# nekStab/neklab

Measured on AMD Instinct MI355X. Metric: linop matvecs/sec + Arnoldi iter time, E=10k N=7, 1/2/4/8 GPU, higher is better.
Workload: dtype f64

## Files before the change

neklab_amd/csrc/lns.hip:

```cpp
#include <cmath>
#include <functional>
#include <map>
#include <string>

#include "internal.h"

using namespace nlg;

namespace {

constexpr int NT = 256;
constexpr int NB = 512;

struct F3 {
    double *p[3];
};
struct CF3 {
    const double *p[3];
};
__device__ __forceinline__ int64_t lane_lo(int64_t ld) { return (int64_t)blockIdx.y * ld; }
__device__ __forceinline__ F3 lane_f3(F3 a, int64_t lo) {
#pragma unroll
    for (int c = 0; c < 3; ++c)
        if (a.p[c]) a.p[c] += lo;
// ... 2003 lines not shown
}

int begin_run(nlg_linop *op, int nl) {
    NLG_TRY(reset_state(op, nl));
    op->istep = 0;
    op->nproj = 0;
    for (int v = 0; v < kMaxLanes; ++v) op->lane_viters[v] = op->lane_piters[v] = 0;
    op->orbit_end_valid = op->upo_fdot_valid = false;
    return 0;
}

int load_state(nlg_linop *op, int lane, const nlg_vec *v, int irst) {
    nlg_mesh *m = op->mesh;
    hipStream_t st = m->ctx->stream;
    for (int c = 0; c < m->dim; ++c)
        NLG_HIP(hipMemcpyAsync(at_lane(op, op->ubuf[0][c], lane), v->vel(c, irst), sizeof(double) * (size_t)m->lvn, hipMemcpyDeviceToDevice, st));
    NLG_HIP(hipMemcpyAsync(at_lane(op, op->p, lane), v->pr(irst), sizeof(double) * (size_t)m->lpn, hipMemcpyDeviceToDevice, st));
    if (op->cfg.ifheat)
        NLG_HIP(hipMemcpyAsync(at_lane(op, op->tbuf[0], lane), v->theta(0, irst), sizeof(double) * (size_t)m->lvn, hipMemcpyDeviceToDevice, st));
    return 0;
}

int store_state(nlg_linop *op, int lane, nlg_vec *v, int irst) {
    nlg_mesh *m = op->mesh;
    hipStream_t st = m->ctx->stream;
    for (int c = 0; c < m->dim; ++c)
        NLG_HIP(hipMemcpyAsync(v->vel(c, irst), at_lane(op, op->ubuf[0][c], lane), sizeof(double) * (size_t)m->lvn, hipMemcpyDeviceToDevice, st));
    NLG_HIP(hipMemcpyAsync(v->pr(irst), at_lane(op, op->p, lane), sizeof(double) * (size_t)m->lpn, hipMemcpyDeviceToDevice, st));
    if (op->cfg.ifheat)
        NLG_HIP(hipMemcpyAsync(v->theta(0, irst), at_lane(op, op->tbuf[0], lane), sizeof(double) * (size_t)m->lvn, hipMemcpyDeviceToDevice, st));
    return 0;
}

int state_minus_x0(nlg_linop *op, int lane, double c, nlg_vec *out) {
    nlg_mesh *m = op->mesh;
    const int dim = m->dim;
    DdtArgs A;
    memset(&A, 0, sizeof(A));
    for (int f = 0; f <= dim; ++f) {
        const bool pr = f == dim;
        A.out[f] = pr ? out->pr() : out->vel(f), A.n[f] = pr ? m->lpn : m->lvn;
        A.src[f][0] = at_lane(op, pr ? op->p : op->ubuf[0][f], lane), A.c[f][0] = c;
        A.src[f][1] = pr ? op->baseflow->pr() : op->baseflow->vel(f), A.c[f][1] = -c;
    }
    NLG_LAUNCH(k_bdf_ddt, dim3(grid_for(m->lvn), dim + 1), dim3(NT), 0, m->ctx->stream, A);
    NLG_HIP(hipGetLastError());
    return 0;
}

enum { FDOT_START = 0, FDOT_PRE, FDOT_END };
int capture_fdot(nlg_linop *op, int lane, int phase) {
    nlg_mesh *m = op->mesh;
    const int dim = m->dim;
    const double idt = 1.0 / op->dt;
    if (phase == FDOT_START) return state_minus_x0(op, lane, idt, op->upo_f0);
    nlg_vec *o = op->upo_fT;
    DdtArgs A;
    memset(&A, 0, sizeof(A));
    for (int c = 0; c < dim; ++c) A.out[c] = o->vel(c), A.n[c] = m->lvn;
    A.out[dim] = o->pr(), A.n[dim] = m->lpn;
    if (phase == FDOT_PRE) {
        const int k = std::min(op->nsteps, op->cfg.torder);
        for (int c = 0; c < dim; ++c)
            for (int j = 0; j < k; ++j) A.src[c][j] = at_lane(op, op->ubuf[j][c], lane), A.c[c][j] = -BDF_C[k][j] * idt;
    } else {
        const int k = std::min(op->nsteps, op->cfg.torder);
// ... 68 lines not shown
    for (int v = 0; v < s; ++v) {
        NLG_CHECK(vin[v] && vout[v] && vin[v]->mesh == m && vout[v]->mesh == m, "exptA block matvec: vector %d NULL or on a different mesh", v);
        NLG_CHECK(vin[v]->nscal == want_scal && vout[v]->nscal == want_scal, "exptA block matvec: vector %d carries %d scalars, the operator %d", v,
                  vin[v]->nscal, want_scal);
        NLG_CHECK(op->cfg.no_history || (vin[v]->lorder >= op->cfg.torder && vout[v]->lorder >= op->cfg.torder), "exptA block matvec: vector lorder < time order");
        for (int u = 0; u < s; ++u) NLG_CHECK(vin[v] != vout[u], "exptA block matvec: an input vector is also an output vector");
        for (int u = 0; u < v; ++u) NLG_CHECK(vout[v] != vout[u], "exptA block matvec: the same output vector twice");
    }
    const int nrst = op->cfg.no_history ? 0 : op->cfg.torder - 1;
    const int nl = op->orbit ? s + 1 : s, lb = op->orbit ? s : -1;
    NLG_CHECK(op->proj_lanes == 0 || s <= op->proj_lanes, "exptA block matvec: %d vectors on an operator with %d wavenumber lanes (nlg_linop_set_projection_lanes)", s,
              op->proj_lanes);
    const unsigned all = (1u << s) - 1u;
    NLG_TRY(begin_run(op, nl));
    for (int v = 0; v < s; ++v) NLG_TRY(load_state(op, v, vin[v], 0));
    NLG_TRY(project_alpha(op, s, 0, all));
    if (lb >= 0) NLG_TRY(load_state(op, lb, op->baseflow, 0));
    Lanes L{op, nl, lb};
    L.adjoint = adjoint;
    NLG_TRY(run_steps(L, lb, [&](int istep) -> int {
        if (istep <= nrst) {
            unsigned replayed = 0;
            for (int v = 0; v < s; ++v)
                if (vin[v]->nrst > 0) {
                    NLG_TRY(load_state(op, v, vin[v], istep));
                    replayed |= 1u << v;
                }
            if (replayed) NLG_TRY(project_alpha(op, s, 0, replayed));
        }
        return 0;
    }));
    for (int slot = 0; slot < 3; ++slot) NLG_TRY(project_alpha(op, s, slot, all));
    for (int v = 0; v < s; ++v) {
        NLG_TRY(nlg_vec_zero(vout[v]));
        NLG_TRY(store_state(op, v, vout[v], 0));
    }
    if (lb >= 0) {
        NLG_TRY(nlg_vec_zero(op->orbit_end));
        NLG_TRY(store_state(op, lb, op->orbit_end, 0));
        op->orbit_end_valid = true;
    }
    for (int irst = 1; irst <= nrst; ++irst) {
        NLG_TRY(advance(L));
        for (int v = 0; v < s; ++v) {
            NLG_TRY(store_state(op, v, vout[v], irst));
            vout[v]->nrst = std::max(vout[v]->nrst, irst);
        }
    }
    op->st_matvecs += s;
    return 0;
}

int do_matvec(nlg_linop *op, const nlg_vec *vin, nlg_vec *vout, int adjoint) {
    NLG_CHECK(op && vin && vout, "exptA matvec: NULL argument");
    NLG_CHECK(op->inited, "exptA matvec: nlg_linop_init has not been called (reference: exptA%%init(), 1cyl.usr:20)");
    nlg_mesh *m = op->mesh;
    NLG_CHECK(vin->mesh == m && vout->mesh == m,
              "exptA matvec: vector on a different mesh (reference: type_error, exponential_propagator.f90:53-58)");
    NLG_CHECK(vin->nscal == (op->cfg.ifheat ? 1 : 0) && vout->nscal == vin->nscal,
              "exptA matvec: the vectors carry %d scalar(s), the operator expects %d (cfg.ifheat)", vin->nscal, op->cfg.ifheat ? 1 : 0);
    NLG_CHECK(op->cfg.no_history || (vin->lorder >= op->cfg.torder && vout->lorder >= op->cfg.torder),
              "exptA matvec: vector lorder %d < time order %d", vin->lorder, op->cfg.torder);
    NLG_CHECK(vin != vout, "exptA matvec: vec_in and vec_out must be distinct (intent(in) / intent(out))");
    return do_matvec_block(op, 1, &vin, &vout, adjoint);
}

int do_integrate_forced_block(nlg_linop *op, int s, const nlg_vec *const *ic, const nlg_vec *const *f_re, const nlg_vec *const *f_im, double omega,
                              int adjoint, nlg_vec *const *vout) {
    NLG_CHECK(op && f_re && vout, "integrate_forced: NULL argument");
    NLG_CHECK(s >= 1 && s <= kMaxLanes, "integrate_forced: %d forcings unsupported (1..%d)", s, kMaxLanes);
    NLG_CHECK(op->inited, "integrate_forced: nlg_linop_init has not been called");
    NLG_NO_OTD(op, "integrate_forced");
    NLG_CHECK(!op->orbit, "integrate_forced: not available in orbit mode (the forced response about a time-periodic base flow is not built; nlg_linop_set_orbit)");
    NLG_CHECK(op->proj_lanes == 0, "integrate_forced: not available on an operator with wavenumber lanes (a forced run does not project; nlg_linop_set_projection_lanes)");
    nlg_mesh *m = op->mesh;
    Lanes L{op, s};
    for (int v = 0; v < s; ++v) {
        NLG_CHECK(f_re[v] && vout[v], "integrate_forced: NULL argument (forcing or output of lane %d)", v);
        L.f_re[v] = f_re[v];
        L.f_im[v] = f_im ? f_im[v] : nullptr;
    }
    for (int v = 0; v < s; ++v) {
        const nlg_vec *icv = ic ? ic[v] : nullptr;
        NLG_CHECK(L.f_re[v]->mesh == m && vout[v]->mesh == m && (!icv || icv->mesh == m) && (!L.f_im[v] || L.f_im[v]->mesh == m),
                  "integrate_forced: vector on a different mesh");
        for (int u = 0; u < s; ++u)
            NLG_CHECK(vout[v] != L.f_re[u] && vout[v] != L.f_im[u] && !(ic && vout[v] == ic[u]), "integrate_forced: the output must be distinct from the inputs");
        for (int u = 0; u < v; ++u) NLG_CHECK(vout[v] != vout[u], "integrate_forced: the same output vector twice");
        NLG_CHECK(L.f_re[v]->nscal == 0 && vout[v]->nscal == 0, "integrate_forced: scalar (temperature) coupling is not built yet");
    }
    hipStream_t st = m->ctx->stream;
    NLG_TRY(begin_run(op, s));
    for (int v = 0; v < s; ++v) {
        NLG_HIP(hipMemsetAsync(at_lane(op, op->p, v), 0, sizeof(double) * (size_t)m->lps, st));
        if (ic && ic[v]) NLG_TRY(load_state(op, v, ic[v], 0));
    }
    L.adjoint = adjoint;
    L.omega = omega, L.sign = adjoint ? -1.0 : 1.0;
    NLG_TRY(run_steps(L));
    for (int v = 0; v < s; ++v) {
        NLG_TRY(nlg_vec_zero(vout[v]));
        NLG_TRY(store_state(op, v, vout[v], 0));
    }
    return 0;
}

int do_integrate_forced(nlg_linop *op, const nlg_vec *ic, const nlg_vec *f_re, const nlg_vec *f_im, double omega, int adjoint, nlg_vec *vout) {
    NLG_CHECK(op && f_re && vout, "integrate_forced: NULL argument");
    return do_integrate_forced_block(op, 1, &ic, &f_re, &f_im, omega, adjoint, &vout);
}

int do_nonlinear_map(nlg_linop *op, const nlg_vec *vin, nlg_vec *vout) {
    NLG_CHECK(op && vin && vout, "nonlinear_map: NULL argument");
    NLG_NO_OTD(op, "nonlinear_map");
    nlg_mesh *m = op->mesh;
    NLG_CHECK(vin->mesh == m && vout->mesh == m, "nonlinear_map: vector on a different mesh (reference: type_error, fixed_point.f90:31-36)");
    NLG_CHECK(vin->nscal == (op->cfg.ifheat ? 1 : 0) && vout->nscal == vin->nscal,
              "nonlinear_map: the vectors carry %d scalar(s), the operator expects %d (cfg.ifheat)", vin->nscal, op->cfg.ifheat ? 1 : 0);
    NLG_CHECK(vin != vout, "nonlinear_map: vec_in and vec_out must be distinct");
    NLG_CHECK(!op->orbit, "nonlinear_map: the operator is in orbit mode and holds X0 as its base flow (use a second operator, or nlg_linop_set_orbit(op, NULL, 0))");
    NLG_TRY(nlg_vec_copy(op->baseflow, vin));
    NLG_TRY(nlg_linop_init(op));
    NLG_TRY(begin_run(op, 1));
    NLG_TRY(load_state(op, 0, vin, 0));
    Lanes L{op, 1};
    L.nonlinear = 1;
    NLG_TRY(run_steps(L));
    NLG_TRY(nlg_vec_zero(vout));
    NLG_TRY(store_state(op, 0, vout, 0));
    NLG_TRY(nlg_vec_axpby(-1.0, vin, 1.0, vout));
    return 0;
}

}

namespace nlg {
int linop_proj_lanes(const nlg_linop *op) { return op->proj_lanes; }
}

extern "C" {

int nlg_exptA_config_default(nlg_exptA_config *c) {
    NLG_CHECK(c, "nlg_exptA_config_default: NULL");
    memset(c, 0, sizeof(*c));
    c->tau = 1.0;
    c->re = 100.0;
    c->cfl_limit = 0.5;
    c->vtol = 1e-9;
    c->ptol = 1e-7;
    c->dt = 0.0;
    c->torder = 3;
    c->maxit_v = 200;
    c->maxit_p = 2000;
    c->ifheat = 0;
    c->conductivity = 1.0;
    c->rhocp = 1.0;
    c->pproj = 1;
    c->no_history = 0;
    c->filter_weight = 0.0;
    c->filter_modes = 0;
    return 0;
// ... 747 lines not shown
```

neklab_amd/csrc/vec.hip:

```cpp
#include <algorithm>

#include "internal.h"

using namespace nlg;

namespace {

constexpr int NT = 256;

__device__ __forceinline__ double wave_sum(double v) {
#pragma unroll
    for (int o = 32; o > 0; o >>= 1) v += __shfl_down(v, o, 64);
    return v;
}

__device__ __forceinline__ double block_sum(double v, double *sm) {
    v = wave_sum(v);
    const int lane = threadIdx.x & 63, wid = threadIdx.x >> 6;
    __syncthreads();
    if (lane == 0) sm[wid] = v;
    __syncthreads();
    double r = 0.0;
    if (threadIdx.x == 0) {
        const int nw = (blockDim.x + 63) >> 6;
        for (int i = 0; i < nw; ++i) r += sm[i];
    }
    return r;
}

__global__ __launch_bounds__(NT) void k_fill(double2 *x, double v, int64_t n2) {
    for (int64_t i = blockIdx.x * (int64_t)NT + threadIdx.x; i < n2; i += (int64_t)gridDim.x * NT) x[i] = make_double2(v, v);
}

__global__ __launch_bounds__(NT) void k_copy(double2 *y, const double2 *x, int64_t n2) {
    for (int64_t i = blockIdx.x * (int64_t)NT + threadIdx.x; i < n2; i += (int64_t)gridDim.x * NT) y[i] = x[i];
}

__global__ __launch_bounds__(NT) void k_scal(double2 *x, double a, int64_t n2) {
    for (int64_t i = blockIdx.x * (int64_t)NT + threadIdx.x; i < n2; i += (int64_t)gridDim.x * NT) {
        double2 v = x[i];
        v.x = __dmul_rn(v.x, a);
        v.y = __dmul_rn(v.y, a);
        x[i] = v;
    }
}

struct LaneVW {
    const double *V[kMaxLanes];
    double *w[kMaxLanes];
    int nrst[kMaxLanes];
};
struct LaneAB {
    const double *a[kMaxLanes], *b[kMaxLanes];
};

__global__ __launch_bounds__(NT) void k_scal_dev(LaneVW P, const double *q, int64_t n2) {
    const int l = blockIdx.y;
    const double sv = q[l];
    const double a = sv > 0.0 ? 1.0 / sqrt(sv) : 0.0;
    const int64_t n2all = n2 * (1 + P.nrst[l]);
    double2 *x = reinterpret_cast<double2 *>(P.w[l]);
    for (int64_t i = blockIdx.x * (int64_t)NT + threadIdx.x; i < n2all; i += (int64_t)gridDim.x * NT) {
        double2 v = x[i];
        v.x = __dmul_rn(v.x, a);
        v.y = __dmul_rn(v.y, a);
        x[i] = v;
    }
}

__global__ __launch_bounds__(NT) void k_axpby(double2 *y, const double2 *x, double a, double b, int64_t n2,
                                              int nrst, int64_t blk2, int consistent) {
    for (int64_t i = blockIdx.x * (int64_t)NT + threadIdx.x; i < n2; i += (int64_t)gridDim.x * NT) {
        const double2 xv = x[i];
        const double ax0 = __dmul_rn(a, xv.x), ax1 = __dmul_rn(a, xv.y);
        double2 yv = y[i];
        yv.x = __dadd_rn(__dmul_rn(yv.x, b), ax0);
        yv.y = __dadd_rn(__dmul_rn(yv.y, b), ax1);
        y[i] = yv;
        for (int r = 1; r <= nrst; ++r) {
            double2 rv = y[i + r * blk2];
            double s0 = ax0, s1 = ax1;
            if (consistent) {
                const double2 xr = x[i + r * blk2];
                s0 = __dmul_rn(a, xr.x);
                s1 = __dmul_rn(a, xr.y);
            }
            rv.x = __dadd_rn(__dmul_rn(rv.x, b), s0);
            rv.y = __dadd_rn(__dmul_rn(rv.y, b), s1);
            y[i + r * blk2] = rv;
        }
    }
}

// ... 30 lines not shown
    const double2 *f2 = reinterpret_cast<const double2 *>(f0 + off);
    const double2 *m2 = reinterpret_cast<const double2 *>(bm1);
    double acc = 0.0;
    for (int64_t i = beg + threadIdx.x; i < end; i += NT) {
        const double2 vv = v2[i], tv = t2[i];
        double2 wv = w2[i];
        wv.x = __dadd_rn(__dadd_rn(wv.x, -vv.x), __dmul_rn(t, tv.x));
        wv.y = __dadd_rn(__dadd_rn(wv.y, -vv.y), __dmul_rn(t, tv.y));
        w2[i] = wv;
        if (ip) {
            const double2 fv = f2[i], mv = m2[i];
            acc += vv.x * fv.x * mv.x + vv.y * fv.y * mv.y;
        }
    }
    if (ip) {
        const double s = block_sum(acc, sm);
        if (threadIdx.x == 0) partial[c * nblk + blockIdx.x] = s;
    }
}

__global__ __launch_bounds__(NT) void k_reduce_rows(const double *partial, int nper, double *out, int accumulate,
                                                    double *out2) {
    __shared__ double sm[4];
    const double *p = partial + (int64_t)blockIdx.x * nper;
    double acc = 0.0;
    for (int i = threadIdx.x; i < nper; i += NT) acc += p[i];
    const double s = block_sum(acc, sm);
    if (threadIdx.x == 0) {
        out[blockIdx.x] = s;
        if (accumulate) out2[blockIdx.x] += s;
    }
}

template <int KB>
__global__ __launch_bounds__(NT) void k_block_dot(LaneVW P, int64_t vstride, int k, int ncomp, const double *bm1, int64_t lvs, int nblk,
                                                  int nper, double *partial) {
    __shared__ double sm[4 * KB];
    const int l = blockIdx.y / ncomp, c = blockIdx.y - l * ncomp;
    const double *V = P.V[l];
    const double *w = P.w[l];
    const int j0 = blockIdx.z * KB;
    const int kc = (k - j0 < KB) ? (k - j0) : KB;
    const int64_t n2 = lvs >> 1;
    const int64_t per = (n2 + nblk - 1) / nblk;
    const int64_t beg = blockIdx.x * per, end = (beg + per < n2) ? beg + per : n2;
    const double2 *w2 = reinterpret_cast<const double2 *>(w + c * lvs);
    const double2 *m2 = reinterpret_cast<const double2 *>(bm1);
    const double2 *v2[KB];
#pragma unroll
    for (int j = 0; j < KB; ++j) {
        const int jj = (j < kc) ? j : 0;
        v2[j] = reinterpret_cast<const double2 *>(V + (int64_t)(j0 + jj) * vstride + c * lvs);
    }
    double acc[KB];
#pragma unroll
    for (int j = 0; j < KB; ++j) acc[j] = 0.0;
    for (int64_t i = beg + threadIdx.x; i < end; i += NT) {
        const double2 wv = w2[i], mv = m2[i];
        const double x0 = wv.x * mv.x, x1 = wv.y * mv.y;
        double2 vv[KB];
#pragma unroll
        for (int j = 0; j < KB; ++j) vv[j] = v2[j][i];
#pragma unroll
        for (int j = 0; j < KB; ++j) acc[j] += vv[j].x * x0 + vv[j].y * x1;
    }
    const int lane = threadIdx.x & 63, wid = threadIdx.x >> 6;
#pragma unroll
    for (int j = 0; j < KB; ++j) {
        const double s = wave_sum(acc[j]);
        if (lane == 0) sm[wid * KB + j] = s;
    }
    __syncthreads();
    if (threadIdx.x < kc) {
        const int j = threadIdx.x;
        const double s = sm[j] + sm[KB + j] + sm[2 * KB + j] + sm[3 * KB + j];
        partial[((int64_t)l * k + j0 + j) * nper + c * nblk + blockIdx.x] = s;
    }
}

template <int KMAX>
__global__ __launch_bounds__(NT) void k_block_axpy_dot(const double *__restrict__ V, int64_t vstride, int k,
                                                       const double *__restrict__ h, double *__restrict__ w,
                                                       const double *__restrict__ bm1, int64_t lvs, int64_t nv,
                                                       double *__restrict__ partial) {
    __shared__ double sh[KMAX];
    __shared__ double sm[4][KMAX];
    for (int j = threadIdx.x; j < KMAX; j += NT) sh[j] = j < k ? h[j] : 0.0;
    __syncthreads();
    double acc[KMAX];
#pragma unroll
    for (int j = 0; j < KMAX; ++j) acc[j] = 0.0;
    for (int64_t i = blockIdx.x * (int64_t)NT + threadIdx.x; i < nv; i += (int64_t)gridDim.x * NT) {
        double v[KMAX];
#pragma unroll
        for (int j = 0; j < KMAX; ++j) v[j] = j < k ? V[(int64_t)j * vstride + i] : 0.0;
        double s = 0.0;
#pragma unroll
        for (int j = 0; j < KMAX; ++j) s += sh[j] * v[j];
        const double wn = w[i] - s;
        w[i] = wn;
        const double x = wn * bm1[i % lvs];
#pragma unroll
        for (int j = 0; j < KMAX; ++j) acc[j] += v[j] * x;
    }
    const int lane = threadIdx.x & 63, wid = threadIdx.x >> 6;
#pragma unroll
    for (int j = 0; j < KMAX; ++j) {
        const double t = wave_sum(acc[j]);
        if (lane == 0) sm[wid][j] = t;
// ... 27 lines not shown
        double s1 = 0.0;
#pragma unroll
        for (int j = 0; j < KH; ++j) {
            s1 += sh[KH + j] * v[j];
            mine[j * NT] = v[j];
        }
#pragma unroll
        for (int j = 0; j < KH; ++j) v[j] = V[(int64_t)j * vstride + i];
        double s0 = 0.0;
#pragma unroll
        for (int j = 0; j < KH; ++j) s0 += sh[j] * v[j];
        const double wn = w[i] - (s0 + s1);
        w[i] = wn;
        const double x = wn * bm1[i % lvs];
#pragma unroll
        for (int j = 0; j < KH; ++j) {
            acc0[j] += v[j] * x;
            acc1[j] += mine[j * NT] * x;
        }
    }
    const int lane = threadIdx.x & 63, wid = threadIdx.x >> 6;
#pragma unroll
    for (int j = 0; j < KH; ++j) {
        const double t0 = wave_sum(acc0[j]), t1 = wave_sum(acc1[j]);
        if (lane == 0) sm[wid][j] = t0, sm[wid][KH + j] = t1;
    }
    __syncthreads();
    if (threadIdx.x < k) {
        const int j = threadIdx.x;
        partial[(int64_t)j * gridDim.x + blockIdx.x] = (sm[0][j] + sm[1][j]) + (sm[2][j] + sm[3][j]);
    }
}

enum { HIST_NONE = 0, HIST_SWEEP = 1, HIST_MAIN = 2 };
__global__ __launch_bounds__(NT) void k_block_axpy(LaneVW P, int64_t vstride, int k, const double *h, const double *hh, int64_t n2,
                                                   int hist, double sign) {
    extern __shared__ double sh0[];
    double *sh1 = sh0 + k;
    const int l = blockIdx.y;
    h += (int64_t)l * k;
    if (hh) hh += (int64_t)l * k;
    for (int j = threadIdx.x; j < k; j += NT) {
        sh0[j] = h[j];
        sh1[j] = hh ? hh[j] : h[j];
    }
    __syncthreads();
    const int64_t n2all = hist == HIST_SWEEP ? n2 * (1 + P.nrst[l]) : n2;
    const int ncopy = hist == HIST_MAIN ? P.nrst[l] : 0;
    double2 *w2 = reinterpret_cast<double2 *>(P.w[l]);
    const double2 *V2 = reinterpret_cast<const double2 *>(P.V[l]);
    const int64_t vs2 = vstride >> 1;
    for (int64_t i = blockIdx.x * (int64_t)NT + threadIdx.x; i < n2all; i += (int64_t)gridDim.x * NT) {
        const double *sh = (hh && i >= n2) ? sh1 : sh0;
        double s0 = 0.0, s1 = 0.0;
        const double2 *v = V2 + i;
        int j = 0;
        for (; j + 8 <= k; j += 8) {
            double2 t[8];
#pragma unroll
            for (int u = 0; u < 8; ++u) t[u] = v[(int64_t)(j + u) * vs2];
#pragma unroll
            for (int u = 0; u < 8; ++u) {
                s0 += sh[j + u] * t[u].x;
                s1 += sh[j + u] * t[u].y;
            }
        }
        for (; j < k; ++j) {
            const double2 t = v[(int64_t)j * vs2];
            s0 += sh[j] * t.x;
            s1 += sh[j] * t.y;
        }
        double2 wv = w2[i];
        wv.x += sign * s0;
        wv.y += sign * s1;
        w2[i] = wv;
        for (int r = 1; r <= ncopy; ++r) {
            double2 rv = w2[i + r * n2];
            rv.x += sign * s0;
            rv.y += sign * s1;
            w2[i + r * n2] = rv;
        }
    }
}

template <int KB, int S>
__global__ __launch_bounds__(NT) void k_block_dot_s(const double *V, int64_t vstride, int k, const double *W, int64_t wstride,
                                                    const double *bm1, int64_t lvs, int nblk, int nper, double *partial) {
    __shared__ double sm[4 * KB * S];
    const int c = blockIdx.y;
    const int j0 = blockIdx.z * KB;
    const int kc = (k - j0 < KB) ? (k - j0) : KB;
    const int64_t n2 = lvs >> 1;
    const int64_t per = (n2 + nblk - 1) / nblk;
    const int64_t beg = blockIdx.x * per, end = (beg + per < n2) ? beg + per : n2;
    const double2 *m2 = reinterpret_cast<const double2 *>(bm1);
    const double2 *v2[KB];
#pragma unroll
    for (int j = 0; j < KB; ++j) {
        const int jj = (j < kc) ? j : 0;
        v2[j] = reinterpret_cast<const double2 *>(V + (int64_t)(j0 + jj) * vstride + c * lvs);
    }
    double acc[KB][S];
#pragma unroll
    for (int j = 0; j < KB; ++j)
#pragma unroll
        for (int v = 0; v < S; ++v) acc[j][v] = 0.0;
    for (int64_t i = beg + threadIdx.x; i < end; i += NT) {
        const double2 mv = m2[i];
        double x0[S], x1[S];
#pragma unroll
        for (int v = 0; v < S; ++v) {
            const double2 wv = reinterpret_cast<const double2 *>(W + (int64_t)v * wstride + c * lvs)[i];
            x0[v] = wv.x * mv.x;
            x1[v] = wv.y * mv.y;
        }
        double2 vv[KB];
#pragma unroll
        for (int j = 0; j < KB; ++j) vv[j] = v2[j][i];
#pragma unroll
        for (int j = 0; j < KB; ++j)
#pragma unroll
            for (int v = 0; v < S; ++v) acc[j][v] += vv[j].x * x0[v] + vv[j].y * x1[v];
    }
    const int lane = threadIdx.x & 63, wid = threadIdx.x >> 6;
#pragma unroll
    for (int j = 0; j < KB; ++j)
#pragma unroll
        for (int v = 0; v < S; ++v) {
            const double t = wave_sum(acc[j][v]);
            if (lane == 0) sm[wid * KB * S + j * S + v] = t;
        }
    __syncthreads();
    if (threadIdx.x < kc * S) {
        const int q = threadIdx.x;
        const double t = (sm[q] + sm[KB * S + q]) + (sm[2 * KB * S + q] + sm[3 * KB * S + q]);
        partial[((int64_t)j0 * S + q) * nper + c * nblk + blockIdx.x] = t;
    }
}

template <int S>
__global__ __launch_bounds__(NT) void k_block_axpy_s(const double *V, int64_t vstride, int k, const double *h, const double *hh,
                                                     double *W, int64_t wstride, int64_t n2, int64_t blk2, double sign) {
    extern __shared__ double shs[];
    double *sh0 = shs, *sh1 = shs + (size_t)k * S;
    for (int j = threadIdx.x; j < k * S; j += NT) {
        sh0[j] = h[j];
        sh1[j] = hh ? hh[j] : h[j];
    }
    __syncthreads();
    const int64_t vs2 = vstride >> 1, ws2 = wstride >> 1;
    double2 *w2 = reinterpret_cast<double2 *>(W);
    for (int64_t i = blockIdx.x * (int64_t)NT + threadIdx.x; i < n2; i += (int64_t)gridDim.x * NT) {
        const double *sh = (hh && i >= blk2) ? sh1 : sh0;
        const double2 *v = reinterpret_cast<const double2 *>(V) + i;
        double s0[S], s1[S];
#pragma unroll
        for (int q = 0; q < S; ++q) s0[q] = s1[q] = 0.0;
        int j = 0;
        for (; j + 8 <= k; j += 8) {
            double2 t[8];
#pragma unroll
            for (int u = 0; u < 8; ++u) t[u] = v[(int64_t)(j + u) * vs2];
#pragma unroll
            for (int u = 0; u < 8; ++u)
#pragma unroll
                for (int q = 0; q < S; ++q) {
                    s0[q] += sh[(j + u) * S + q] * t[u].x;
                    s1[q] += sh[(j + u) * S + q] * t[u].y;
                }
        }
        for (; j < k; ++j) {
            const double2 t = v[(int64_t)j * vs2];
#pragma unroll
            for (int q = 0; q < S; ++q) {
                s0[q] += sh[j * S + q] * t.x;
                s1[q] += sh[j * S + q] * t.y;
            }
        }
#pragma unroll
        for (int q = 0; q < S; ++q) {
            double2 wv = w2[i + q * ws2];
            wv.x += sign * s0[q];
            wv.y += sign * s1[q];
            w2[i + q * ws2] = wv;
        }
    }
}

template <int S>
__global__ __launch_bounds__(NT) void k_block_rmul(double *W, int64_t wstride, const double *T, int64_t n2) {
    double t[S][S];
#pragma unroll
    for (int a = 0; a < S; ++a)
#pragma unroll
        for (int b = 0; b < S; ++b) t[a][b] = T[a * S + b];
    const int64_t ws2 = wstride >> 1;
    double2 *w2 = reinterpret_cast<double2 *>(W);
    for (int64_t i = blockIdx.x * (int64_t)NT + threadIdx.x; i < n2; i += (int64_t)gridDim.x * NT) {
        double2 x[S], y[S];
#pragma unroll
        for (int a = 0; a < S; ++a) x[a] = w2[i + a * ws2];
#pragma unroll
        for (int b = 0; b < S; ++b) {
            y[b].x = y[b].y = 0.0;
#pragma unroll
// ... 441 lines not shown
    if (ctx->distributed()) {
        NLG_LAUNCH(k_reduce_rows, dim3(rows), dim3(NT), 0, st, ctx->d_partial, per, out, 0, (double *)nullptr);
        NLG_TRY(allreduce_sum(ctx, out, rows));
        if (acc) NLG_LAUNCH(k_vadd, dim3((rows + 255) / 256), dim3(256), 0, st, acc, out, rows);
    } else {
        ++g_collectives;
        NLG_LAUNCH(k_reduce_rows, dim3(rows), dim3(NT), 0, st, ctx->d_partial, per, out, acc ? 1 : 0, acc);
    }
    return 0;
}

static LaneVW lanes_of(int s, const nlg_basis *const *b, nlg_vec *const *w) {
    LaneVW P;
    for (int l = 0; l < kMaxLanes; ++l) {
        const int u = l < s ? l : 0;
        P.V[l] = b[u]->d, P.w[l] = w[u]->d, P.nrst[l] = w[u]->nrst;
    }
    return P;
}
static LaneVW one_lane(const nlg_basis *b, const nlg_vec *w) {
    nlg_vec *wl = const_cast<nlg_vec *>(w);
    return lanes_of(1, &b, &wl);
}
static int max_nrst(int s, const LaneVW &P) { return *std::max_element(P.nrst, P.nrst + s); }

static int lanes_block_dot(const nlg_basis *b0, int s, const LaneVW &P, int k, double *d_out, double *d_acc) {
    nlg_mesh *m = b0->mesh;
    nlg_ctx *ctx = m->ctx;
    const nlg_vec *v0 = b0->views[0];
    constexpr int KB = 8;
    const int nblk = dot_nblk(v0), nper = nblk * v0->ncomp;
    NLG_TRY(reduce_ws_reserve(ctx, s * k));
    ProfScope ps(ctx, P_BLOCKDOT);
    NLG_LAUNCH(k_block_dot<KB>, dim3(nblk, v0->ncomp * s, (k + KB - 1) / KB), dim3(NT), 0, ctx->stream, P, b0->stride, k, v0->ncomp,
               (const double *)m->d_bm1, m->lvs, nblk, nper, ctx->d_partial);
    NLG_TRY(reduce_rows_all(ctx, s * k, nper, d_out, d_acc));
    NLG_HIP(hipGetLastError());
    return 0;
}

static int lanes_block_axpy(const nlg_basis *b0, int s, const LaneVW &P, int k, const double *d_h, const double *d_hh, int hist,
                            double sign) {
    nlg_ctx *ctx = b0->mesh->ctx;
    const int64_t n2 = b0->views[0]->main_len / 2;
    const int64_t n2all = hist == HIST_SWEEP ? n2 * (1 + max_nrst(s, P)) : n2;
    ProfScope ps(ctx, P_BLOCKAXPY);
    NLG_LAUNCH(k_block_axpy, dim3(grid_for(n2all), s), dim3(NT), sizeof(double) * 2 * k, ctx->stream, P, b0->stride, k, d_h, d_hh, n2,
               hist, sign);
    NLG_HIP(hipGetLastError());
    return 0;
}

static int hist_mode() { return g_axpby_consistent ? HIST_SWEEP : HIST_MAIN; }

static int cgs2_fused_sweep(const nlg_basis *b, int k, nlg_vec *w, double *h, double *h2) {
    nlg_ctx *ctx = b->mesh->ctx;
    const nlg_vec *v0 = b->views[0];
    const LaneVW P = one_lane(b, w);
    const int kf = std::min(k, 128);
    const int k0 = k - kf;
    const int64_t nv = (int64_t)v0->ncomp * b->mesh->lvs;
    const int G = 256;
    NLG_TRY(reduce_ws_reserve(ctx, k));
    if (k0 > 0) NLG_TRY(lanes_block_axpy(b, 1, P, k0, h, nullptr, HIST_NONE, -1.0));
    const double *Vf = b->d + (int64_t)k0 * b->stride;
    {
        ProfScope ps(ctx, P_AXPYDOT);
        if (kf > 64) {
            constexpr size_t lds2 = sizeof(double) * (2 * 64 + 64 * NT);
            static bool attr_set = false;
            if (!attr_set) {
                NLG_HIP(hipFuncSetAttribute(reinterpret_cast<const void *>(&k_block_axpy_dot2<64>), hipFuncAttributeMaxDynamicSharedMemorySize, (int)lds2));
                attr_set = true;
            }
            NLG_LAUNCH(k_block_axpy_dot2<64>, dim3(G), dim3(NT), lds2, ctx->stream, Vf, b->stride, kf, (const double *)(h + k0), w->d,
                       (const double *)b->mesh->d_bm1, b->mesh->lvs, nv, ctx->d_partial);
        } else {
            NLG_LAUNCH(k_block_axpy_dot<64>, dim3(G), dim3(NT), 0, ctx->stream, Vf, b->stride, kf, (const double *)(h + k0), w->d,
                       (const double *)b->mesh->d_bm1, b->mesh->lvs, nv, ctx->d_partial);
        }
    }
    {
        ProfScope ps(ctx, P_BLOCKAXPY);
        const int64_t np2 = (w->main_len - nv) / 2;
        if (np2 > 0) {
            LaneVW Pp = {};
            Pp.V[0] = Vf + nv, Pp.w[0] = w->d + nv;
            NLG_LAUNCH(k_block_axpy, dim3(grid_for(np2)), dim3(NT), sizeof(double) * 2 * kf, ctx->stream, Pp, b->stride, kf,
                       (const double *)(h + k0), (const double *)nullptr, np2, (int)HIST_NONE, -1.0);
        }
    }
    NLG_TRY(reduce_rows_all(ctx, kf, G, h2 + k0, h + k0));
    if (k0 > 0) NLG_TRY(lanes_block_dot(b, 1, P, k0, h2, h));
    return 0;
}

static int basis_cgs2_dev(int s, nlg_basis *const *b, int k, nlg_vec *const *w) {
    nlg_basis *b0 = b[0];
    nlg_mesh *m = b0->mesh;
    nlg_ctx *ctx = m->ctx;
    double *H1 = b0->h1(), *H2 = b0->h2(), *Q = b0->hnorm(s, k);
    const LaneVW P = lanes_of(s, b, w);
    if (k > 0) {
        NLG_TRY(lanes_block_dot(b0, s, P, k, H1, nullptr));
        if (g_axpby_consistent) {
            if (s == 1 && k >= 24) {
                NLG_TRY(cgs2_fused_sweep(b0, k, w[0], H1, H2));
            } else {
                NLG_TRY(lanes_block_axpy(b0, s, P, k, H1, nullptr, HIST_NONE, -1.0));
                NLG_TRY(lanes_block_dot(b0, s, P, k, H2, H1));
            }
            NLG_TRY(lanes_block_axpy(b0, s, P, k, H2, H1, HIST_SWEEP, -1.0));
        } else {
            NLG_TRY(lanes_block_axpy(b0, s, P, k, H1, nullptr, HIST_MAIN, -1.0));
            NLG_TRY(lanes_block_dot(b0, s, P, k, H2, H1));
            NLG_TRY(lanes_block_axpy(b0, s, P, k, H2, nullptr, HIST_MAIN, -1.0));
        }
    }
    const nlg_vec *v0 = b0->views[0];
    const int nblk = dot_nblk(v0), nper = nblk * v0->ncomp;
    const int64_t n2 = v0->main_len / 2;
    LaneAB A;
    for (int l = 0; l < kMaxLanes; ++l) A.a[l] = A.b[l] = P.w[l];
    NLG_LAUNCH(k_dot_partial, dim3(nblk, v0->ncomp, s), dim3(NT), 0, ctx->stream, A, (const double *)m->d_bm1, m->lvs, nblk, nper,
               ctx->d_partial);
    NLG_TRY(reduce_rows_all(ctx, s, nper, Q, nullptr));
    NLG_LAUNCH(k_scal_dev, dim3(grid_for(n2 * (1 + max_nrst(s, P))), s), dim3(NT), 0, ctx->stream, P, (const double *)Q, n2);
    NLG_HIP(hipGetLastError());
    return 0;
}

int basis_cgs2_host(int s, nlg_basis *const *b, int k, nlg_vec *const *w, double *h, int64_t hstride, double *beta, int64_t bstride) {
    NLG_TRY(basis_cgs2_dev(s, b, k, w));
    std::vector<double> tmp((size_t)s * k + s);
    hipStream_t st = b[0]->mesh->ctx->stream;
    NLG_HIP(hipMemcpyAsync(tmp.data(), b[0]->h1(), sizeof(double) * tmp.size(), hipMemcpyDeviceToHost, st));
    NLG_HIP(hipStreamSynchronize(st));
    for (int l = 0; l < s; ++l) {
        for (int j = 0; j < k; ++j) h[l * hstride + j] = tmp[(size_t)l * k + j];
        beta[l * bstride] = sqrt(tmp[(size_t)s * k + l]);
    }
    return 0;
}

}

extern "C" {

int nlg_basis_cgs2_batch(int s, nlg_basis *const *b, int k, nlg_vec *const *w, double *h, int ldh, double *beta) {
    NLG_CHECK(b && w && h && beta, "nlg_basis_cgs2_batch: NULL argument");
    NLG_CHECK(s >= 1 && s <= kMaxLanes, "nlg_basis_cgs2_batch: %d lanes unsupported (1..%d)", s, kMaxLanes);
    for (int l = 0; l < s; ++l) NLG_CHECK(b[l] && w[l], "nlg_basis_cgs2_batch: NULL basis or vector in lane %d", l);
    NLG_CHECK(k >= 0 && k <= b[0]->nvec, "nlg_basis_cgs2_batch: k=%d out of range [0,%d]", k, b[0]->nvec);
    NLG_CHECK(ldh >= k, "nlg_basis_cgs2_batch: ldh=%d too small for k=%d", ldh, k);
    for (int l = 0; l < s; ++l) {
        NLG_CHECK(b[l]->mesh == b[0]->mesh && b[l]->nscal == b[0]->nscal && b[l]->lorder == b[0]->lorder && b[l]->nvec == b[0]->nvec,
                  "nlg_basis_cgs2_batch: the bases differ in shape (lane %d)", l);
        NLG_TRY(check_same(b[l]->views[0], w[l], "nlg_basis_cgs2_batch"));
        for (int u = 0; u < l; ++u) NLG_CHECK(b[l] != b[u] && w[l] != w[u], "nlg_basis_cgs2_batch: the same basis or vector in two lanes");
        for (int u = 0; u < s; ++u)
// ... 66 lines not shown
    NLG_CHECK(b && coef, "nlg_basis_block_cgs2: NULL argument");
    NLG_CHECK(s >= 1 && s <= 4, "nlg_basis_block_cgs2: block size %d unsupported (1..4)", s);
    NLG_CHECK(k >= 0 && k + s <= b->nvec, "nlg_basis_block_cgs2: columns %d..%d outside the basis (nvec=%d)", k, k + s - 1, b->nvec);
    NLG_CHECK(g_axpby_consistent, "nlg_basis_block_cgs2: the block path implements the consistent restart-history update only");
    nlg_ctx *ctx = b->mesh->ctx;
    hipStream_t st = ctx->stream;
    const int ld = k + s;
    if (s == 1) {
        std::vector<double> h(std::max(k, 1));
        double beta = 0.0;
        NLG_TRY(nlg_basis_cgs2(b, k, b->views[k], h.data(), &beta));
        for (int j = 0; j < k; ++j) coef[j] = h[j];
        coef[k] = beta;
        return 0;
    }
    nlg_vec *w0 = b->views[k];
    int nrst = 0;
    for (int v = 0; v < s; ++v) nrst = std::max(nrst, b->views[k + v]->nrst);
    for (int v = 0; v < s; ++v) {
        nlg_vec *c = b->views[k + v];
        if (c->nrst < nrst)
            NLG_HIP(hipMemsetAsync(c->d + (int64_t)(1 + c->nrst) * c->main_len, 0, sizeof(double) * (size_t)((nrst - c->nrst) * c->main_len), st));
        c->nrst = nrst;
    }
    b->last_block_rank = s;
    double *W = w0->d;
    double *H1 = b->h1(), *H2 = b->h2(), *dG = b->gram(), *dT = b->tmat();
    const int nblk = dot_nblk(w0), nper = nblk * w0->ncomp;
    const int64_t n2 = w0->main_len / 2, n2all = n2 * (1 + nrst);
    constexpr int KB = 8;
    NLG_TRY(reduce_ws_reserve(ctx, std::max(k, s) * s));
    auto dots = [&](const double *V, int kk, double *out, double *acc) -> int {
        ProfScope ps(ctx, P_BLOCKDOT);
        const dim3 g(nblk, w0->ncomp, (kk + KB - 1) / KB);
#define BD(S_) NLG_LAUNCH((k_block_dot_s<KB, S_>), g, dim3(NT), 0, st, V, b->stride, kk, (const double *)W, b->stride, \
                                  (const double *)b->mesh->d_bm1, b->mesh->lvs, nblk, nper, ctx->d_partial)
        if (s == 2) BD(2);
        else if (s == 3) BD(3);
        else BD(4);
#undef BD
        return nlg::reduce_rows_all(ctx, kk * s, nper, out, acc);
    };
    auto axpy = [&](const double *h, const double *hh, int64_t n, int64_t blk2) -> int {
        ProfScope ps(ctx, P_BLOCKAXPY);
        const size_t lds = sizeof(double) * 2 * (size_t)k * s;
#define BA(S_) NLG_LAUNCH((k_block_axpy_s<S_>), dim3(grid_for(n)), dim3(NT), lds, st, (const double *)b->d, b->stride, k, h, hh, W, \
                                  b->stride, n, blk2, -1.0)
        if (s == 2) BA(2);
        else if (s == 3) BA(3);
        else BA(4);
#undef BA
        return 0;
    };
    if (k > 0) {
        NLG_TRY(dots(b->d, k, H1, nullptr));
        NLG_TRY(axpy(H1, nullptr, n2, n2));
        NLG_TRY(dots(b->d, k, H2, H1));
        NLG_TRY(axpy(H2, H1, n2all, n2));
    }
    double R[4][4] = {};
    for (int a = 0; a < s; ++a) R[a][a] = 1.0;
    bool dep[4] = {false, false, false, false};
    double hsq[4] = {0.0, 0.0, 0.0, 0.0};
    std::vector<double> hs((size_t)std::max(k, 1) * s);
    if (k > 0) {
        NLG_HIP(hipMemcpyAsync(hs.data(), H1, sizeof(double) * (size_t)k * s, hipMemcpyDeviceToHost, st));
        NLG_HIP(hipStreamSynchronize(st));
// ... 92 lines not shown
```

Before: 24.56.

## Add nontemporal basis loads, XCD-aware dot tiling, fused history tail axpy, partial output clears

Basis-vector loads in the block dot and axpy kernels become nontemporal when the basis exceeds about 1 GiB, so streamed data does not evict cache. The dot grids are flattened so adjacent chunks share an XCD while all tiles of a chunk are visited. In the CGS2 path the history part of the second axpy is deferred and fused with the final normalisation, and the scale kernel then touches only the main segment. Full zeroing of output vectors before a store is replaced by clearing only the unfilled tail. This adds template variants and moves the history correction after the norm, which could change rounding order.

Result: faster. 25.03, median of 6 (+1.9%).

```diff
diff --git a/neklab_amd/csrc/lns.hip b/neklab_amd/csrc/lns.hip
--- a/neklab_amd/csrc/lns.hip
+++ b/neklab_amd/csrc/lns.hip
@@ -2059,6 +2059,14 @@
     return 0;
 }
 
+int clear_for_store(nlg_vec *v, int nfill) {
+    const int ntail = v->lorder - 1 - nfill;
+    if (ntail > 0)
+        NLG_HIP(hipMemsetAsync(v->d + (int64_t)(1 + nfill) * v->main_len, 0, sizeof(double) * (size_t)(ntail * v->main_len), v->mesh->ctx->stream));
+    v->nrst = 0;
+    return 0;
+}
+
 int state_minus_x0(nlg_linop *op, int lane, double c, nlg_vec *out) {
     nlg_mesh *m = op->mesh;
     const int dim = m->dim;
@@ -2193,11 +2201,11 @@
     }));
     for (int slot = 0; slot < 3; ++slot) NLG_TRY(project_alpha(op, s, slot, all));
     for (int v = 0; v < s; ++v) {
-        NLG_TRY(nlg_vec_zero(vout[v]));
+        NLG_TRY(clear_for_store(vout[v], nrst));
         NLG_TRY(store_state(op, v, vout[v], 0));
     }
     if (lb >= 0) {
-        NLG_TRY(nlg_vec_zero(op->orbit_end));
+        NLG_TRY(clear_for_store(op->orbit_end, 0));
         NLG_TRY(store_state(op, lb, op->orbit_end, 0));
         op->orbit_end_valid = true;
     }
@@ -2260,7 +2268,7 @@
     L.omega = omega, L.sign = adjoint ? -1.0 : 1.0;
     NLG_TRY(run_steps(L));
     for (int v = 0; v < s; ++v) {
-        NLG_TRY(nlg_vec_zero(vout[v]));
+        NLG_TRY(clear_for_store(vout[v], 0));
         NLG_TRY(store_state(op, v, vout[v], 0));
     }
     return 0;
@@ -2287,7 +2295,7 @@
     Lanes L{op, 1};
     L.nonlinear = 1;
     NLG_TRY(run_steps(L));
-    NLG_TRY(nlg_vec_zero(vout));
+    NLG_TRY(clear_for_store(vout, 0));
     NLG_TRY(store_state(op, 0, vout, 0));
     NLG_TRY(nlg_vec_axpby(-1.0, vin, 1.0, vout));
     return 0;
diff --git a/neklab_amd/csrc/vec.hip b/neklab_amd/csrc/vec.hip
--- a/neklab_amd/csrc/vec.hip
+++ b/neklab_amd/csrc/vec.hip
@@ -28,6 +28,15 @@
     return r;
 }
 
+template <bool NTL = true>
+__device__ __forceinline__ double2 ld_once(const double2 *p) {
+    if (!NTL) return *p;
+    typedef double v2d __attribute__((ext_vector_type(2)));
+    const v2d t = __builtin_nontemporal_load(reinterpret_cast<const v2d *>(p));
+    return make_double2(t.x, t.y);
+}
+inline bool stream_basis(int k, int64_t len) { return (int64_t)k * len * (int64_t)sizeof(double) >= ((int64_t)1 << 30); }
+
 __global__ __launch_bounds__(NT) void k_fill(double2 *x, double v, int64_t n2) {
     for (int64_t i = blockIdx.x * (int64_t)NT + threadIdx.x; i < n2; i += (int64_t)gridDim.x * NT) x[i] = make_double2(v, v);
 }
@@ -54,11 +63,12 @@
     const double *a[kMaxLanes], *b[kMaxLanes];
 };
 
-__global__ __launch_bounds__(NT) void k_scal_dev(LaneVW P, const double *q, int64_t n2) {
+__device__ __forceinline__ double inv_norm(double sv) { return sv > 0.0 ? 1.0 / sqrt(sv) : 0.0; }
+
+__global__ __launch_bounds__(NT) void k_scal_dev(LaneVW P, const double *q, int64_t n2, int hist) {
     const int l = blockIdx.y;
-    const double sv = q[l];
-    const double a = sv > 0.0 ? 1.0 / sqrt(sv) : 0.0;
-    const int64_t n2all = n2 * (1 + P.nrst[l]);
+    const double a = inv_norm(q[l]);
+    const int64_t n2all = hist ? n2 * (1 + P.nrst[l]) : n2;
     double2 *x = reinterpret_cast<double2 *>(P.w[l]);
     for (int64_t i = blockIdx.x * (int64_t)NT + threadIdx.x; i < n2all; i += (int64_t)gridDim.x * NT) {
         double2 v = x[i];
@@ -155,18 +165,29 @@
     }
 }
 
-template <int KB>
+constexpr int kXcd = 8;
+inline unsigned chunk_tile_grid(int nblk, int ntile) { return (unsigned)((nblk + kXcd - 1) / kXcd * kXcd * ntile); }
+__device__ __forceinline__ void chunk_tile(int ntile, int &chunk, int &tile) {
+    const int grp = blockIdx.x / (kXcd * ntile), rem = blockIdx.x - grp * kXcd * ntile;
+    chunk = grp * kXcd + rem % kXcd;
+    tile = rem / kXcd;
+}
+
+template <int KB, bool NTL>
 __global__ __launch_bounds__(NT) void k_block_dot(LaneVW P, int64_t vstride, int k, int ncomp, const double *bm1, int64_t lvs, int nblk,
                                                   int nper, double *partial) {
     __shared__ double sm[4 * KB];
     const int l = blockIdx.y / ncomp, c = blockIdx.y - l * ncomp;
     const double *V = P.V[l];
     const double *w = P.w[l];
-    const int j0 = blockIdx.z * KB;
+    int chunk, tile;
+    chunk_tile((k + KB - 1) / KB, chunk, tile);
+    if (chunk >= nblk) return;
+    const int j0 = tile * KB;
     const int kc = (k - j0 < KB) ? (k - j0) : KB;
     const int64_t n2 = lvs >> 1;
     const int64_t per = (n2 + nblk - 1) / nblk;
-    const int64_t beg = blockIdx.x * per, end = (beg + per < n2) ? beg + per : n2;
+    const int64_t beg = chunk * per, end = (beg + per < n2) ? beg + per : n2;
     const double2 *w2 = reinterpret_cast<const double2 *>(w + c * lvs);
     const double2 *m2 = reinterpret_cast<const double2 *>(bm1);
     const double2 *v2[KB];
@@ -183,7 +204,7 @@
         const double x0 = wv.x * mv.x, x1 = wv.y * mv.y;
         double2 vv[KB];
 #pragma unroll
-        for (int j = 0; j < KB; ++j) vv[j] = v2[j][i];
+        for (int j = 0; j < KB; ++j) vv[j] = ld_once<NTL>(v2[j] + i);
 #pragma unroll
         for (int j = 0; j < KB; ++j) acc[j] += vv[j].x * x0 + vv[j].y * x1;
     }
@@ -197,7 +218,7 @@
     if (threadIdx.x < kc) {
         const int j = threadIdx.x;
         const double s = sm[j] + sm[KB + j] + sm[2 * KB + j] + sm[3 * KB + j];
-        partial[((int64_t)l * k + j0 + j) * nper + c * nblk + blockIdx.x] = s;
+        partial[((int64_t)l * k + j0 + j) * nper + c * nblk + chunk] = s;
     }
 }
 
@@ -291,12 +312,14 @@
     }
 }
 
-enum { HIST_NONE = 0, HIST_SWEEP = 1, HIST_MAIN = 2 };
+enum { HIST_NONE = 0, HIST_SWEEP = 1, HIST_MAIN = 2, HIST_ONLY = 3 };
+template <bool TAIL, bool NTL>
 __global__ __launch_bounds__(NT) void k_block_axpy(LaneVW P, int64_t vstride, int k, const double *h, const double *hh, int64_t n2,
-                                                   int hist, double sign) {
+                                                   int hist, double sign, const double *q) {
     extern __shared__ double sh0[];
     double *sh1 = sh0 + k;
     const int l = blockIdx.y;
+    if (TAIL && P.nrst[l] == 0) return;
     h += (int64_t)l * k;
     if (hh) hh += (int64_t)l * k;
     for (int j = threadIdx.x; j < k; j += NT) {
@@ -304,12 +327,14 @@
         sh1[j] = hh ? hh[j] : h[j];
     }
     __syncthreads();
-    const int64_t n2all = hist == HIST_SWEEP ? n2 * (1 + P.nrst[l]) : n2;
-    const int ncopy = hist == HIST_MAIN ? P.nrst[l] : 0;
+    const int64_t n2all = (TAIL || hist == HIST_SWEEP) ? n2 * (1 + P.nrst[l]) : n2;
+    const int64_t ibeg = TAIL ? n2 : 0;
+    const int ncopy = (!TAIL && hist == HIST_MAIN) ? P.nrst[l] : 0;
+    const double a = TAIL ? inv_norm(q[l]) : 1.0;
     double2 *w2 = reinterpret_cast<double2 *>(P.w[l]);
     const double2 *V2 = reinterpret_cast<const double2 *>(P.V[l]);
     const int64_t vs2 = vstride >> 1;
-    for (int64_t i = blockIdx.x * (int64_t)NT + threadIdx.x; i < n2all; i += (int64_t)gridDim.x * NT) {
+    for (int64_t i = ibeg + blockIdx.x * (int64_t)NT + threadIdx.x; i < n2all; i += (int64_t)gridDim.x * NT) {
         const double *sh = (hh && i >= n2) ? sh1 : sh0;
         double s0 = 0.0, s1 = 0.0;
         const double2 *v = V2 + i;
@@ -317,7 +342,7 @@
         for (; j + 8 <= k; j += 8) {
             double2 t[8];
 #pragma unroll
-            for (int u = 0; u < 8; ++u) t[u] = v[(int64_t)(j + u) * vs2];
+            for (int u = 0; u < 8; ++u) t[u] = ld_once<NTL>(v + (int64_t)(j + u) * vs2);
 #pragma unroll
             for (int u = 0; u < 8; ++u) {
                 s0 += sh[j + u] * t[u].x;
@@ -325,13 +350,17 @@
             }
         }
         for (; j < k; ++j) {
-            const double2 t = v[(int64_t)j * vs2];
+            const double2 t = ld_once<NTL>(v + (int64_t)j * vs2);
             s0 += sh[j] * t.x;
             s1 += sh[j] * t.y;
         }
         double2 wv = w2[i];
         wv.x += sign * s0;
         wv.y += sign * s1;
+        if (TAIL) {
+            wv.x = __dmul_rn(wv.x, a);
+            wv.y = __dmul_rn(wv.y, a);
+        }
         w2[i] = wv;
         for (int r = 1; r <= ncopy; ++r) {
             double2 rv = w2[i + r * n2];
@@ -347,11 +376,14 @@
                                                     const double *bm1, int64_t lvs, int nblk, int nper, double *partial) {
     __shared__ double sm[4 * KB * S];
     const int c = blockIdx.y;
-    const int j0 = blockIdx.z * KB;
+    int chunk, tile;
+    chunk_tile((k + KB - 1) / KB, chunk, tile);
+    if (chunk >= nblk) return;
+    const int j0 = tile * KB;
     const int kc = (k - j0 < KB) ? (k - j0) : KB;
     const int64_t n2 = lvs >> 1;
     const int64_t per = (n2 + nblk - 1) / nblk;
-    const int64_t beg = blockIdx.x * per, end = (beg + per < n2) ? beg + per : n2;
+    const int64_t beg = chunk * per, end = (beg + per < n2) ? beg + per : n2;
     const double2 *m2 = reinterpret_cast<const double2 *>(bm1);
     const double2 *v2[KB];
 #pragma unroll
@@ -375,7 +407,7 @@
         }
         double2 vv[KB];
 #pragma unroll
-        for (int j = 0; j < KB; ++j) vv[j] = v2[j][i];
+        for (int j = 0; j < KB; ++j) vv[j] = ld_once(v2[j] + i);
 #pragma unroll
         for (int j = 0; j < KB; ++j)
 #pragma unroll
@@ -393,7 +425,7 @@
     if (threadIdx.x < kc * S) {
         const int q = threadIdx.x;
         const double t = (sm[q] + sm[KB * S + q]) + (sm[2 * KB * S + q] + sm[3 * KB * S + q]);
-        partial[((int64_t)j0 * S + q) * nper + c * nblk + blockIdx.x] = t;
+        partial[((int64_t)j0 * S + q) * nper + c * nblk + chunk] = t;
     }
 }
 
@@ -419,7 +451,7 @@
         for (; j + 8 <= k; j += 8) {
             double2 t[8];
 #pragma unroll
-            for (int u = 0; u < 8; ++u) t[u] = v[(int64_t)(j + u) * vs2];
+            for (int u = 0; u < 8; ++u) t[u] = ld_once(v + (int64_t)(j + u) * vs2);
 #pragma unroll
             for (int u = 0; u < 8; ++u)
 #pragma unroll
@@ -429,7 +461,7 @@
                 }
         }
         for (; j < k; ++j) {
-            const double2 t = v[(int64_t)j * vs2];
+            const double2 t = ld_once(v + (int64_t)j * vs2);
 #pragma unroll
             for (int q = 0; q < S; ++q) {
                 s0[q] += sh[j * S + q] * t.x;
@@ -937,21 +969,37 @@
     const int nblk = dot_nblk(v0), nper = nblk * v0->ncomp;
     NLG_TRY(reduce_ws_reserve(ctx, s * k));
     ProfScope ps(ctx, P_BLOCKDOT);
-    NLG_LAUNCH(k_block_dot<KB>, dim3(nblk, v0->ncomp * s, (k + KB - 1) / KB), dim3(NT), 0, ctx->stream, P, b0->stride, k, v0->ncomp,
-               (const double *)m->d_bm1, m->lvs, nblk, nper, ctx->d_partial);
+    const dim3 g(chunk_tile_grid(nblk, (k + KB - 1) / KB), v0->ncomp * s);
+    if (stream_basis(k, v0->main_len))
+        NLG_LAUNCH((k_block_dot<KB, true>), g, dim3(NT), 0, ctx->stream, P, b0->stride, k, v0->ncomp, (const double *)m->d_bm1, m->lvs, nblk,
+                   nper, ctx->d_partial);
+    else
+        NLG_LAUNCH((k_block_dot<KB, false>), g, dim3(NT), 0, ctx->stream, P, b0->stride, k, v0->ncomp, (const double *)m->d_bm1, m->lvs, nblk,
+                   nper, ctx->d_partial);
     NLG_TRY(reduce_rows_all(ctx, s * k, nper, d_out, d_acc));
     NLG_HIP(hipGetLastError());
     return 0;
 }
 
 static int lanes_block_axpy(const nlg_basis *b0, int s, const LaneVW &P, int k, const double *d_h, const double *d_hh, int hist,
-                            double sign) {
+                            double sign, const double *d_q = nullptr) {
     nlg_ctx *ctx = b0->mesh->ctx;
     const int64_t n2 = b0->views[0]->main_len / 2;
-    const int64_t n2all = hist == HIST_SWEEP ? n2 * (1 + max_nrst(s, P)) : n2;
+    const int mr = max_nrst(s, P);
+    if (hist == HIST_ONLY && mr == 0) return 0;
+    const int64_t n2all = hist == HIST_SWEEP ? n2 * (1 + mr) : hist == HIST_ONLY ? n2 * mr : n2;
     ProfScope ps(ctx, P_BLOCKAXPY);
-    NLG_LAUNCH(k_block_axpy, dim3(grid_for(n2all), s), dim3(NT), sizeof(double) * 2 * k, ctx->stream, P, b0->stride, k, d_h, d_hh, n2,
-               hist, sign);
+    const bool ntl = stream_basis(k, 2 * n2);
+#define BAX(T_, N_) NLG_LAUNCH((k_block_axpy<T_, N_>), dim3(grid_for(n2all), s), dim3(NT), sizeof(double) * 2 * k, ctx->stream, P, b0->stride, k, \
+                               d_h, d_hh, n2, hist, sign, d_q)
+    if (hist == HIST_ONLY) {
+        if (ntl) BAX(true, true);
+        else BAX(true, false);
+    } else {
+        if (ntl) BAX(false, true);
+        else BAX(false, false);
+    }
+#undef BAX
     NLG_HIP(hipGetLastError());
     return 0;
 }
@@ -991,8 +1039,12 @@
         if (np2 > 0) {
             LaneVW Pp = {};
             Pp.V[0] = Vf + nv, Pp.w[0] = w->d + nv;
-            NLG_LAUNCH(k_block_axpy, dim3(grid_for(np2)), dim3(NT), sizeof(double) * 2 * kf, ctx->stream, Pp, b->stride, kf,
-                       (const double *)(h + k0), (const double *)nullptr, np2, (int)HIST_NONE, -1.0);
+            if (stream_basis(kf, w->main_len))
+                NLG_LAUNCH((k_block_axpy<false, true>), dim3(grid_for(np2)), dim3(NT), sizeof(double) * 2 * kf, ctx->stream, Pp, b->stride, kf,
+                           (const double *)(h + k0), (const double *)nullptr, np2, (int)HIST_NONE, -1.0, (const double *)nullptr);
+            else
+                NLG_LAUNCH((k_block_axpy<false, false>), dim3(grid_for(np2)), dim3(NT), sizeof(double) * 2 * kf, ctx->stream, Pp, b->stride, kf,
+                           (const double *)(h + k0), (const double *)nullptr, np2, (int)HIST_NONE, -1.0, (const double *)nullptr);
         }
     }
     NLG_TRY(reduce_rows_all(ctx, kf, G, h2 + k0, h + k0));
@@ -1006,6 +1058,7 @@
     nlg_ctx *ctx = m->ctx;
     double *H1 = b0->h1(), *H2 = b0->h2(), *Q = b0->hnorm(s, k);
     const LaneVW P = lanes_of(s, b, w);
+    const bool split = k > 0 && g_axpby_consistent;
     if (k > 0) {
         NLG_TRY(lanes_block_dot(b0, s, P, k, H1, nullptr));
         if (g_axpby_consistent) {
@@ -1015,7 +1068,7 @@
                 NLG_TRY(lanes_block_axpy(b0, s, P, k, H1, nullptr, HIST_NONE, -1.0));
                 NLG_TRY(lanes_block_dot(b0, s, P, k, H2, H1));
             }
-            NLG_TRY(lanes_block_axpy(b0, s, P, k, H2, H1, HIST_SWEEP, -1.0));
+            NLG_TRY(lanes_block_axpy(b0, s, P, k, H2, nullptr, HIST_NONE, -1.0));
         } else {
             NLG_TRY(lanes_block_axpy(b0, s, P, k, H1, nullptr, HIST_MAIN, -1.0));
             NLG_TRY(lanes_block_dot(b0, s, P, k, H2, H1));
@@ -1030,7 +1083,9 @@
     NLG_LAUNCH(k_dot_partial, dim3(nblk, v0->ncomp, s), dim3(NT), 0, ctx->stream, A, (const double *)m->d_bm1, m->lvs, nblk, nper,
                ctx->d_partial);
     NLG_TRY(reduce_rows_all(ctx, s, nper, Q, nullptr));
-    NLG_LAUNCH(k_scal_dev, dim3(grid_for(n2 * (1 + max_nrst(s, P))), s), dim3(NT), 0, ctx->stream, P, (const double *)Q, n2);
+    if (split) NLG_TRY(lanes_block_axpy(b0, s, P, k, H1, nullptr, HIST_ONLY, -1.0, Q));
+    NLG_LAUNCH(k_scal_dev, dim3(grid_for(split ? n2 : n2 * (1 + max_nrst(s, P))), s), dim3(NT), 0, ctx->stream, P, (const double *)Q, n2,
+               split ? 0 : 1);
     NLG_HIP(hipGetLastError());
     return 0;
 }
@@ -1163,7 +1218,7 @@
     NLG_TRY(reduce_ws_reserve(ctx, std::max(k, s) * s));
     auto dots = [&](const double *V, int kk, double *out, double *acc) -> int {
         ProfScope ps(ctx, P_BLOCKDOT);
-        const dim3 g(nblk, w0->ncomp, (kk + KB - 1) / KB);
+        const dim3 g(chunk_tile_grid(nblk, (kk + KB - 1) / KB), w0->ncomp);
 #define BD(S_) NLG_LAUNCH((k_block_dot_s<KB, S_>), g, dim3(NT), 0, st, V, b->stride, kk, (const double *)W, b->stride, \
                                   (const double *)b->mesh->d_bm1, b->mesh->lvs, nblk, nper, ctx->d_partial)
         if (s == 2) BD(2);
```
